# nmdl-mizo/lcaonet

Hardware: NVIDIA B200
Metric: molecules/sec fwd+bwd (QM9-shape) (higher is better)
Workload: dtype f32

## Files before the change

### lcaonet_b200/csrc/gemm_tc.cu

```cuda
#include "common.cuh"

namespace {

constexpr int kEpiWarps = 4;
constexpr int kBlockM = 128;
constexpr int kChunkK = 32;
constexpr uint32_t kSpinLimit = 1u << 28;

__device__ __forceinline__ uint32_t smem_u32(const void* p) { return (uint32_t)__cvta_generic_to_shared(p); }

__device__ __forceinline__ void mbar_init(uint64_t* bar, uint32_t count) {
  asm volatile("mbarrier.init.shared::cta.b64 [%0], %1;" ::"r"(smem_u32(bar)), "r"(count));
}
__device__ __forceinline__ void mbar_arrive(uint64_t* bar) {
  asm volatile("mbarrier.arrive.shared::cta.b64 _, [%0];" ::"r"(smem_u32(bar)) : "memory");
}
__device__ __forceinline__ void mbar_wait(uint64_t* bar, uint32_t parity) {
  uint32_t done = 0, spins = 0;
  const uint32_t addr = smem_u32(bar);
  while (!done) {
    asm volatile(
        "{\n\t.reg .pred p;\n\t"
        "mbarrier.try_wait.parity.shared::cta.b64 p, [%1], %2;\n\t"
        "selp.u32 %0, 1, 0, p;\n\t}"
        : "=r"(done)
        : "r"(addr), "r"(parity)
        : "memory");
    if (!done && ++spins > kSpinLimit) __trap();
  }
}
__device__ __forceinline__ void fence_barrier_init() { asm volatile("fence.mbarrier_init.release.cluster;" ::: "memory"); }
__device__ __forceinline__ void fence_proxy_async() { asm volatile("fence.proxy.async.shared::cta;" ::: "memory"); }
__device__ __forceinline__ void tc_fence_before() { asm volatile("tcgen05.fence::before_thread_sync;" ::: "memory"); }
__device__ __forceinline__ void tc_fence_after() { asm volatile("tcgen05.fence::after_thread_sync;" ::: "memory"); }

__device__ __forceinline__ void tmem_alloc(uint32_t* dst_smem, uint32_t ncols) {
  asm volatile("tcgen05.alloc.cta_group::1.sync.aligned.shared::cta.b32 [%0], %1;" ::"r"(smem_u32(dst_smem)), "r"(ncols)
               : "memory");
  asm volatile("tcgen05.relinquish_alloc_permit.cta_group::1.sync.aligned;" ::: "memory");
}
__device__ __forceinline__ void tmem_dealloc(uint32_t taddr, uint32_t ncols) {
  asm volatile("tcgen05.dealloc.cta_group::1.sync.aligned.b32 %0, %1;" ::"r"(taddr), "r"(ncols) : "memory");
}
__device__ __forceinline__ bool elect_one() {
  uint32_t pred;
  asm volatile("{\n\t.reg .pred p;\n\telect.sync _|p, 0xffffffff;\n\tselp.u32 %0, 1, 0, p;\n\t}" : "=r"(pred));
  return pred != 0;
}
__device__ __forceinline__ void umma_tf32(uint32_t tmem_d, uint64_t desc_a, uint64_t desc_b, uint32_t idesc,
                                          uint32_t accumulate) {
  asm volatile(
      "{\n\t.reg .pred p;\n\t"
      "setp.ne.b32 p, %4, 0;\n\t"
      "tcgen05.mma.cta_group::1.kind::tf32 [%0], %1, %2, %3, p;\n\t}"
      ::"r"(tmem_d), "l"(desc_a), "l"(desc_b), "r"(idesc), "r"(accumulate)
      : "memory");
}
__device__ __forceinline__ void umma_commit(uint64_t* bar) {
  asm volatile("tcgen05.commit.cta_group::1.mbarrier::arrive::one.shared::cluster.b64 [%0];" ::"r"(smem_u32(bar))
               : "memory");
}
__device__ __forceinline__ void tmem_ld32(uint32_t taddr, float (&v)[32]) {
  uint32_t r[32];
  asm volatile(
      "tcgen05.ld.sync.aligned.32x32b.x32.b32 "
      "{%0,%1,%2,%3,%4,%5,%6,%7,%8,%9,%10,%11,%12,%13,%14,%15,%16,%17,%18,%19,%20,%21,%22,%23,%24,%25,%26,%27,%28,%29,%30,%31}, [%32];"
      : "=r"(r[0]), "=r"(r[1]), "=r"(r[2]), "=r"(r[3]), "=r"(r[4]), "=r"(r[5]), "=r"(r[6]), "=r"(r[7]), "=r"(r[8]),
        "=r"(r[9]), "=r"(r[10]), "=r"(r[11]), "=r"(r[12]), "=r"(r[13]), "=r"(r[14]), "=r"(r[15]), "=r"(r[16]),
        "=r"(r[17]), "=r"(r[18]), "=r"(r[19]), "=r"(r[20]), "=r"(r[21]), "=r"(r[22]), "=r"(r[23]), "=r"(r[24]),
        "=r"(r[25]), "=r"(r[26]), "=r"(r[27]), "=r"(r[28]), "=r"(r[29]), "=r"(r[30]), "=r"(r[31])
      : "r"(taddr)
      : "memory");
  asm volatile("tcgen05.wait::ld.sync.aligned;" ::: "memory");
#pragma unroll
  for (int i = 0; i < 32; ++i) v[i] = __uint_as_float(r[i]);
}

__device__ __forceinline__ uint64_t make_desc_sw128(uint32_t smem_addr) {
  uint64_t d = 0;
  d |= (uint64_t)((smem_addr & 0x3FFFFu) >> 4);
  d |= (uint64_t)1 << 16;
  d |= (uint64_t)(1024 >> 4) << 32;
  d |= (uint64_t)1 << 46;
  d |= (uint64_t)2 << 61;
  return d;
}
__device__ __forceinline__ uint32_t sw128_off(int row, int chunk) { return row * 128 + ((chunk ^ (row & 7)) << 4); }
__host__ __device__ constexpr uint32_t make_idesc(int M, int N) {
  return (1u << 4) | (2u << 7) | (2u << 10) | ((uint32_t)(N >> 3) << 17) | ((uint32_t)(M >> 4) << 24);
}

__device__ __forceinline__ float tf32_hi(float x) { return __uint_as_float(__float_as_uint(x) & 0xFFFFE000u); }
__device__ __forceinline__ void split4(const float4 x, float4& hi, float4& lo) {
  hi = make_float4(tf32_hi(x.x), tf32_hi(x.y), tf32_hi(x.z), tf32_hi(x.w));
  lo = make_float4(tf32_hi(x.x - hi.x), tf32_hi(x.y - hi.y), tf32_hi(x.z - hi.z), tf32_hi(x.w - hi.w));
}
__device__ __forceinline__ float sigmoid_fast(float x) { return __fdividef(1.0f, 1.0f + __expf(-x)); }
__device__ __forceinline__ float silu_fast(float x) { return x * sigmoid_fast(x); }
__device__ __forceinline__ float silu_grad_fast(float x) {
  const float sg = sigmoid_fast(x);
  return sg * fmaf(x, 1.0f - sg, 1.0f);
}
__device__ __forceinline__ float4 silu_grad4(float4 g, float4 h) {
  return make_float4(g.x * silu_grad_fast(h.x), g.y * silu_grad_fast(h.y), g.z * silu_grad_fast(h.z), g.w * silu_grad_fast(h.w));
}

__device__ __forceinline__ void store8(float* p, const float* v, bool wide) {
  if (wide) {
    asm volatile("st.global.v8.f32 [%0], {%1,%2,%3,%4,%5,%6,%7,%8};" ::"l"(p), "f"(v[0]), "f"(v[1]), "f"(v[2]), "f"(v[3]),
                 "f"(v[4]), "f"(v[5]), "f"(v[6]), "f"(v[7])
                 : "memory");
  } else {
    st4(p, make_float4(v[0], v[1], v[2], v[3]));
    st4(p + 4, make_float4(v[4], v[5], v[6], v[7]));
  }
}

struct RowsArgs {
  const float* A; int64_t lda;
  const float* W; int64_t ldw;
  const float* bias;
  const float* G; int64_t ldg;
  float* Y; int64_t ldy;
  float* pre; int64_t ldp;
  int64_t M; int Kc; int Nb;
  int b_trans, act, accumulate, x3, stages, lo_stages;
  int wide_store;
};

constexpr int kLoadWarps = 4;
constexpr int kRowsThreads = (4 + 4 + 1 + kLoadWarps) * 32;
constexpr int kEpiPitch = 144;
constexpr int kEpiWarpBytes = 32 * kEpiPitch;
constexpr uint32_t kStageBytes = kBlockM * 128;

__device__ __forceinline__ void cp_async16(uint32_t dst, const void* src, uint32_t src_bytes) {
  asm volatile("cp.async.cg.shared.global [%0], [%1], 16, %2;" ::"r"(dst), "l"(src), "r"(src_bytes) : "memory");
}
__device__ __forceinline__ void cp_async_arrive(uint64_t* bar) {
  asm volatile("cp.async.mbarrier.arrive.noinc.shared::cta.b64 [%0];" ::"r"(smem_u32(bar)) : "memory");
}

template <bool EPI8>
__global__ void __launch_bounds__(EPI8 ? kRowsThreads + 128 : kRowsThreads, 1) k_tc_rows(const RowsArgs g) {
  extern __shared__ __align__(1024) uint8_t smem_raw[];
  pdl_trigger();
  const int warp = threadIdx.x >> 5, lane = threadIdx.x & 31;
  const uint32_t blockB = g.Nb * 128;
  const uint32_t halfB = (g.Kc / kChunkK) * blockB;
  const int R = g.stages, L = g.lo_stages;
  uint8_t* sB = smem_raw;
  uint8_t* sHi = sB + 2 * halfB;
  uint8_t* sLo = sHi + (size_t)R * kStageBytes;
  uint64_t* bars = reinterpret_cast<uint64_t*>(sLo + (size_t)(g.x3 ? L : 0) * kStageBytes);
  uint64_t* raw_full = bars;
  uint64_t* full = raw_full + R;
  uint64_t* hi_empty = full + R;
  uint64_t* lo_empty = hi_empty + R;
  uint64_t* tfull = lo_empty + L;
  uint64_t* tempty = tfull + 2;
  uint32_t* tmem_slot = reinterpret_cast<uint32_t*>(tempty + 2);

  const int64_t nblocks = (g.M + kBlockM - 1) / kBlockM;
  const int nchunk = g.Kc / kChunkK;
  const uint32_t acc_cols = g.x3 ? 2 * g.Nb : g.Nb;
  const uint32_t need_cols = 2 * acc_cols;
  const uint32_t tmem_cols = need_cols <= 32 ? 32 : need_cols <= 64 ? 64 : need_cols <= 128 ? 128 : need_cols <= 256 ? 256 : 512;

  if (threadIdx.x == 0) {
    for (int s = 0; s < R; ++s) {
      mbar_init(&raw_full[s], kLoadWarps * 32);
      mbar_init(&full[s], 4 * 32);
      mbar_init(&hi_empty[s], 1);
    }
    for (int s = 0; s < L; ++s) mbar_init(&lo_empty[s], 1);
    for (int a = 0; a < 2; ++a) {
      mbar_init(&tfull[a], 1);
      mbar_init(&tempty[a], (EPI8 ? 2 : 1) * kEpiWarps * 32);
    }
    fence_barrier_init();
  }
  if (warp == 8) tmem_alloc(tmem_slot, tmem_cols);
  tc_fence_before();
  __syncthreads();
  tc_fence_after();
  const uint32_t tmem_base = *tmem_slot;

  constexpr int kStageThreads = (4 + 4 + 1) * 32;
  constexpr int kWB = 8;
  if (warp < 9) {
    const int kq = g.Kc / 4, total = g.Nb * kq;
    for (int base = 0; base < total; base += kWB * kStageThreads) {
      float4 w[kWB];
      int n[kWB], kg[kWB];
#pragma unroll
      for (int u = 0; u < kWB; ++u) {
        const int idx = base + u * kStageThreads + (int)threadIdx.x;
        w[u] = make_float4(0.f, 0.f, 0.f, 0.f);
        n[u] = -1;
        if (idx < total) {
          if (!g.b_trans) {
            n[u] = idx / kq; kg[u] = idx - n[u] * kq;
            w[u] = ldg4(g.W + (int64_t)n[u] * g.ldw + kg[u] * 4);
          } else {
            kg[u] = idx / g.Nb; n[u] = idx - kg[u] * g.Nb;
            w[u] = make_float4(__ldg(g.W + (int64_t)(kg[u] * 4 + 0) * g.ldw + n[u]), __ldg(g.W + (int64_t)(kg[u] * 4 + 1) * g.ldw + n[u]),
                               __ldg(g.W + (int64_t)(kg[u] * 4 + 2) * g.ldw + n[u]), __ldg(g.W + (int64_t)(kg[u] * 4 + 3) * g.ldw + n[u]));
          }
        }
      }
#pragma unroll
      for (int u = 0; u < kWB; ++u) {
        if (n[u] >= 0) {
          float4 hi, lo;
          split4(w[u], hi, lo);
          const uint32_t off = (kg[u] >> 3) * blockB + sw128_off(n[u], kg[u] & 7);
          *reinterpret_cast<float4*>(sB + off) = hi;
          *reinterpret_cast<float4*>(sB + halfB + off) = lo;
        }
      }
    }
    fence_proxy_async();
    asm volatile("bar.sync 1, %0;" ::"n"(kStageThreads) : "memory");
  }

  pdl_wait();
  if (warp >= 9 && warp < 13) {
    const int lw = warp - 9, row_in = lane >> 3, c = lane & 7;
    const uint32_t hi_base = smem_u32(sHi);
    uint32_t it = 0;
    for (int64_t mb = blockIdx.x; mb < nblocks; mb += gridDim.x) {
      const int64_t mrow = mb * kBlockM + 32 * lw + row_in;
      for (int kc = 0; kc < nchunk; ++kc, ++it) {
        const int s = it % R;
        mbar_wait(&hi_empty[s], ((it / R) & 1) ^ 1);
        const uint32_t dst = hi_base + s * kStageBytes;
        const float* src = g.A + mrow * g.lda + kc * kChunkK + c * 4;
#pragma unroll
        for (int j = 0; j < 8; ++j) {
          const bool ok = mrow + 4 * j < g.M;
          cp_async16(dst + sw128_off(32 * lw + 4 * j + row_in, c), ok ? src + (int64_t)4 * j * g.lda : g.A, ok ? 16u : 0u);
        }
        cp_async_arrive(&raw_full[s]);
      }
    }
  } else if (warp >= 4 && warp < 8) {
    const int t = threadIdx.x - 128;
    uint32_t it = 0;
    for (int64_t mb = blockIdx.x; mb < nblocks; mb += gridDim.x) {
      for (int kc = 0; kc < nchunk; ++kc, ++it) {
        const int s = it % R, l = it % L;
        mbar_wait(&raw_full[s], (it / R) & 1);
        if (g.x3) {
          mbar_wait(&lo_empty[l], ((it / L) & 1) ^ 1);
          uint8_t* ph = sHi + (size_t)s * kStageBytes + t * 16;
          uint8_t* pl = sLo + (size_t)l * kStageBytes + t * 16;
#pragma unroll
          for (int i = 0; i < 8; ++i) {
            float4 hi, lo;
            split4(*reinterpret_cast<const float4*>(ph + i * 2048), hi, lo);
            *reinterpret_cast<float4*>(ph + i * 2048) = hi;
            *reinterpret_cast<float4*>(pl + i * 2048) = lo;
          }
        }
        fence_proxy_async();
        mbar_arrive(&full[s]);
      }
    }
  } else if (warp == 8) {
    {
      const uint32_t idesc = make_idesc(kBlockM, g.Nb);
      const uint32_t hiBase = smem_u32(sHi), loBase = smem_u32(sLo), bBase = smem_u32(sB);
      uint32_t it = 0, tile = 0;
      for (int64_t mb = blockIdx.x; mb < nblocks; mb += gridDim.x, ++tile) {
        const int acc = tile & 1;
        mbar_wait(&tempty[acc], ((tile >> 1) & 1) ^ 1);
        tc_fence_after();
        const uint32_t d = tmem_base + acc * acc_cols, dc = d + g.Nb;
        for (int kc = 0; kc < nchunk; ++kc, ++it) {
          const int s = it % R, l = it % L;
          mbar_wait(&full[s], (it / R) & 1);
          tc_fence_after();
          const uint32_t a_hi = hiBase + s * kStageBytes, a_lo = loBase + l * kStageBytes;
          const uint32_t b_hi = bBase + kc * blockB, b_lo = b_hi + halfB;
          const uint64_t dAh0 = make_desc_sw128(a_hi), dBh0 = make_desc_sw128(b_hi), dAl0 = make_desc_sw128(a_lo), dBl0 = make_desc_sw128(b_lo);
#pragma unroll
          for (int kk = 0; kk < kChunkK / 8; ++kk) {
            const uint64_t dAh = dAh0 + 2 * kk, dBh = dBh0 + 2 * kk, dAl = dAl0 + 2 * kk, dBl = dBl0 + 2 * kk;
            if (elect_one()) {
              umma_tf32(d, dAh, dBh, idesc, (kc | kk) != 0);
              if (g.x3) {
                umma_tf32(dc, dAl, dBh, idesc, (kc | kk) != 0);
                umma_tf32(dc, dAh, dBl, idesc, 1);
              }
            }
          }
          if (elect_one()) {
            umma_commit(&hi_empty[s]);
            if (g.x3) umma_commit(&lo_empty[l]);
          }
        }
        if (elect_one()) umma_commit(&tfull[acc]);
      }
    }
    __syncwarp();
  } else {
    const bool wide = g.wide_store != 0;
    const int quad = warp & 3;
    const int c_begin = (EPI8 && warp >= 13) ? 64 : 0, c_end = EPI8 ? min(g.Nb, c_begin + 64) : g.Nb;
    uint32_t tile = 0;
    for (int64_t mb = blockIdx.x; mb < nblocks; mb += gridDim.x, ++tile) {
      const int acc = tile & 1;
      const int64_t m = mb * kBlockM + quad * 32 + lane;
      float4 gq[8];
      if (g.G && m < g.M) {
#pragma unroll
        for (int q = 0; q < 8; ++q)
          gq[q] = (c_begin + 4 * q < g.Nb) ? ldg4(g.G + m * g.ldg + c_begin + 4 * q) : make_float4(0.f, 0.f, 0.f, 0.f);
      }
      mbar_wait(&tfull[acc], (tile >> 1) & 1);
      tc_fence_after();
      for (int c0 = c_begin; c0 < c_end; c0 += 32) {
        float4 gn[8];
        if (g.G && m < g.M && c0 + 32 < c_end) {
#pragma unroll
          for (int q = 0; q < 8; ++q)
            gn[q] = (c0 + 32 + 4 * q < g.Nb) ? ldg4(g.G + m * g.ldg + c0 + 32 + 4 * q) : make_float4(0.f, 0.f, 0.f, 0.f);
        }
        float v[32];
        tmem_ld32(tmem_base + ((uint32_t)(quad * 32) << 16) + acc * acc_cols + c0, v);
        if (g.x3) {
          float w[32];
          tmem_ld32(tmem_base + ((uint32_t)(quad * 32) << 16) + acc * acc_cols + g.Nb + c0, w);
#pragma unroll
          for (int j = 0; j < 32; ++j) v[j] += w[j];
        }
        if (m < g.M) {
          const int nc = min(32, g.Nb - c0);
#pragma unroll
          for (int j = 0; j < 32; j += 8) {
            if (j < nc) {
              float* o = v + j;
              if (g.bias) {
                const float4 b0 = ldg4(g.bias + c0 + j), b1 = ldg4(g.bias + c0 + j + 4);
                o[0] += b0.x; o[1] += b0.y; o[2] += b0.z; o[3] += b0.w; o[4] += b1.x; o[5] += b1.y; o[6] += b1.z; o[7] += b1.w;
              }
              if (g.accumulate) {
                const float4 p0 = *reinterpret_cast<const float4*>(g.Y + m * g.ldy + c0 + j);
                const float4 p1 = *reinterpret_cast<const float4*>(g.Y + m * g.ldy + c0 + j + 4);
                o[0] += p0.x; o[1] += p0.y; o[2] += p0.z; o[3] += p0.w; o[4] += p1.x; o[5] += p1.y; o[6] += p1.z; o[7] += p1.w;
              }
              if (g.pre) store8(g.pre + m * g.ldp + c0 + j, o, wide);
              if (g.act == LCAO_ACT_SILU) {
#pragma unroll
                for (int q = 0; q < 8; ++q) o[q] = silu_fast(o[q]);
              }
              if (g.G) {
                const float4 h0 = gq[j / 4], h1 = gq[j / 4 + 1];
                o[0] *= silu_grad_fast(h0.x); o[1] *= silu_grad_fast(h0.y); o[2] *= silu_grad_fast(h0.z); o[3] *= silu_grad_fast(h0.w);
                o[4] *= silu_grad_fast(h1.x); o[5] *= silu_grad_fast(h1.y); o[6] *= silu_grad_fast(h1.z); o[7] *= silu_grad_fast(h1.w);
              }
              store8(g.Y + m * g.ldy + c0 + j, o, wide);
            }
          }
        }
        if (g.G) {
#pragma unroll
          for (int q = 0; q < 8; ++q) gq[q] = gn[q];
        }
      }
      tc_fence_before();
      mbar_arrive(&tempty[acc]);
    }
  }
  tc_fence_before();
  __syncthreads();
  if (warp == 8) {
    tc_fence_after();
    tmem_dealloc(tmem_base, tmem_cols);
  }
}

constexpr int kTaThreads = 15 * 32;
constexpr int kTaStages = 4;
constexpr uint32_t kTaCol0 = 256;

__device__ __forceinline__ void umma_tf32_ts(uint32_t tmem_d, uint32_t tmem_a, uint64_t desc_b, uint32_t idesc, uint32_t accumulate) {
  asm volatile(
      "{\n\t.reg .pred p;\n\t"
      "setp.ne.b32 p, %4, 0;\n\t"
      "tcgen05.mma.cta_group::1.kind::tf32 [%0], [%1], %2, %3, p;\n\t}"
      ::"r"(tmem_d), "r"(tmem_a), "l"(desc_b), "r"(idesc), "r"(accumulate)
      : "memory");
}
__device__ __forceinline__ void tmem_st32(uint32_t taddr, const uint32_t (&r)[32]) {
  asm volatile(
      "tcgen05.st.sync.aligned.32x32b.x32.b32 [%0], "
      "{%1,%2,%3,%4,%5,%6,%7,%8,%9,%10,%11,%12,%13,%14,%15,%16,%17,%18,%19,%20,%21,%22,%23,%24,%25,%26,%27,%28,%29,%30,%31,%32};"
      ::"r"(taddr), "r"(r[0]), "r"(r[1]), "r"(r[2]), "r"(r[3]), "r"(r[4]), "r"(r[5]), "r"(r[6]), "r"(r[7]), "r"(r[8]), "r"(r[9]),
        "r"(r[10]), "r"(r[11]), "r"(r[12]), "r"(r[13]), "r"(r[14]), "r"(r[15]), "r"(r[16]), "r"(r[17]), "r"(r[18]), "r"(r[19]),
        "r"(r[20]), "r"(r[21]), "r"(r[22]), "r"(r[23]), "r"(r[24]), "r"(r[25]), "r"(r[26]), "r"(r[27]), "r"(r[28]), "r"(r[29]),
        "r"(r[30]), "r"(r[31])
      : "memory");
}
__device__ __forceinline__ void tmem_ld32_nw(uint32_t taddr, float (&v)[32]) {
  asm volatile(
      "tcgen05.ld.sync.aligned.32x32b.x32.b32 "
      "{%0,%1,%2,%3,%4,%5,%6,%7,%8,%9,%10,%11,%12,%13,%14,%15,%16,%17,%18,%19,%20,%21,%22,%23,%24,%25,%26,%27,%28,%29,%30,%31}, [%32];"
      : "=f"(v[0]), "=f"(v[1]), "=f"(v[2]), "=f"(v[3]), "=f"(v[4]), "=f"(v[5]), "=f"(v[6]), "=f"(v[7]), "=f"(v[8]),
        "=f"(v[9]), "=f"(v[10]), "=f"(v[11]), "=f"(v[12]), "=f"(v[13]), "=f"(v[14]), "=f"(v[15]), "=f"(v[16]),
        "=f"(v[17]), "=f"(v[18]), "=f"(v[19]), "=f"(v[20]), "=f"(v[21]), "=f"(v[22]), "=f"(v[23]), "=f"(v[24]),
        "=f"(v[25]), "=f"(v[26]), "=f"(v[27]), "=f"(v[28]), "=f"(v[29]), "=f"(v[30]), "=f"(v[31])
      : "r"(taddr)
      : "memory");
}
__device__ __forceinline__ void tmem_wait_ld() { asm volatile("tcgen05.wait::ld.sync.aligned;" ::: "memory"); }
__device__ __forceinline__ void tmem_wait_st() { asm volatile("tcgen05.wait::st.sync.aligned;" ::: "memory"); }

__global__ void __launch_bounds__(kTaThreads, 1) k_tc_rows_ta(const RowsArgs g) {
  constexpr int kLd = 2;
  extern __shared__ __align__(1024) uint8_t smem_raw[];
  pdl_trigger();
  const int warp = threadIdx.x >> 5, lane = threadIdx.x & 31;
  const uint32_t blockB = g.Nb * 128;
  const uint32_t halfB = (g.Kc / kChunkK) * blockB;
  const int R = g.stages;
  uint8_t* sB = smem_raw;
  uint8_t* sRaw = sB + 2 * halfB;
  uint64_t* bars = reinterpret_cast<uint64_t*>(sRaw + (size_t)R * kStageBytes);
  uint64_t* raw_full = bars;
  uint64_t* raw_empty = raw_full + R;
  uint64_t* a_full = raw_empty + R;
  uint64_t* a_empty = a_full + kTaStages;
  uint64_t* tfull = a_empty + kTaStages;
  uint64_t* tempty = tfull + 2;
  uint32_t* tmem_slot = reinterpret_cast<uint32_t*>(tempty + 2);
  const int64_t nblocks = (g.M + kBlockM - 1) / kBlockM;
  const int nchunk = g.Kc / kChunkK;
  constexpr uint32_t tmem_cols = 512;

  if (threadIdx.x == 0) {
    for (int s = 0; s < R; ++s) {
      mbar_init(&raw_full[s], kLd * 32);
      mbar_init(&raw_empty[s], 4 * 32);
    }
    for (int s = 0; s < kTaStages; ++s) {
      mbar_init(&a_full[s], 4 * 32);
      mbar_init(&a_empty[s], 1);
    }
    for (int a = 0; a < 2; ++a) {
      mbar_init(&tfull[a], 1);
      mbar_init(&tempty[a], 2 * kEpiWarps * 32);
    }
    fence_barrier_init();
  }
  if (warp == 8) tmem_alloc(tmem_slot, tmem_cols);
  tc_fence_before();
  __syncthreads();
  tc_fence_after();
  const uint32_t tmem_base = *tmem_slot;

  constexpr int kStageThreads = (4 + 4 + 1) * 32;
  constexpr int kWB = 8;
  if (warp < 9) {
    const int kq = g.Kc / 4, total = g.Nb * kq;
    for (int base = 0; base < total; base += kWB * kStageThreads) {
      float4 w[kWB];
      int n[kWB], kg[kWB];
#pragma unroll
      for (int u = 0; u < kWB; ++u) {
        const int idx = base + u * kStageThreads + (int)threadIdx.x;
        w[u] = make_float4(0.f, 0.f, 0.f, 0.f);
        n[u] = -1;
        if (idx < total) {
          if (!g.b_trans) {
            n[u] = idx / kq; kg[u] = idx - n[u] * kq;
            w[u] = ldg4(g.W + (int64_t)n[u] * g.ldw + kg[u] * 4);
          } else {
            kg[u] = idx / g.Nb; n[u] = idx - kg[u] * g.Nb;
            w[u] = make_float4(__ldg(g.W + (int64_t)(kg[u] * 4 + 0) * g.ldw + n[u]), __ldg(g.W + (int64_t)(kg[u] * 4 + 1) * g.ldw + n[u]),
                               __ldg(g.W + (int64_t)(kg[u] * 4 + 2) * g.ldw + n[u]), __ldg(g.W + (int64_t)(kg[u] * 4 + 3) * g.ldw + n[u]));
          }
        }
      }
#pragma unroll
      for (int u = 0; u < kWB; ++u) {
        if (n[u] >= 0) {
          float4 hi, lo;
          split4(w[u], hi, lo);
          const uint32_t off = (kg[u] >> 3) * blockB + sw128_off(n[u], kg[u] & 7);
          *reinterpret_cast<float4*>(sB + off) = hi;
          *reinterpret_cast<float4*>(sB + halfB + off) = lo;
        }
      }
    }
    fence_proxy_async();
    asm volatile("bar.sync 1, %0;" ::"n"(kStageThreads) : "memory");
  }
  pdl_wait();

  if (warp >= 9 && warp < 9 + kLd) {
    constexpr int kRowsPerLd = kBlockM / kLd;
    const int lw = warp - 9, row_in = lane >> 3, c = lane & 7;
    const uint32_t raw_base = smem_u32(sRaw);
    uint32_t it = 0;
    for (int64_t mb = blockIdx.x; mb < nblocks; mb += gridDim.x) {
      const int64_t mrow = mb * kBlockM + kRowsPerLd * lw + row_in;
      for (int kc = 0; kc < nchunk; ++kc, ++it) {
        const int s = it % R;
        mbar_wait(&raw_empty[s], ((it / R) & 1) ^ 1);
        const uint32_t dst = raw_base + s * kStageBytes;
        const float* src = g.A + mrow * g.lda + kc * kChunkK + c * 4;
#pragma unroll
        for (int j = 0; j < kRowsPerLd / 4; ++j) {
          const bool ok = mrow + 4 * j < g.M;
          cp_async16(dst + sw128_off(kRowsPerLd * lw + 4 * j + row_in, c), ok ? src + (int64_t)4 * j * g.lda : g.A, ok ? 16u : 0u);
        }
        cp_async_arrive(&raw_full[s]);
      }
    }
  } else if (warp >= 4 && warp < 8) {
    const int row = (warp & 3) * 32 + lane;
    const uint32_t lane_base = (uint32_t)((warp & 3) * 32) << 16;
    uint32_t it = 0;
    for (int64_t mb = blockIdx.x; mb < nblocks; mb += gridDim.x) {
      for (int kc = 0; kc < nchunk; ++kc, ++it) {
        const int s = it % R, ts = it % kTaStages;
        mbar_wait(&raw_full[s], (it / R) & 1);
        mbar_wait(&a_empty[ts], ((it / kTaStages) & 1) ^ 1);
        tc_fence_after();
        const uint8_t* pr = sRaw + (size_t)s * kStageBytes;
        uint32_t hi[32], lo[32];
#pragma unroll
        for (int c = 0; c < 8; ++c) {
          const float4 v = *reinterpret_cast<const float4*>(pr + sw128_off(row, c));
          float4 h, l;
          split4(v, h, l);
          hi[4 * c] = __float_as_uint(h.x); hi[4 * c + 1] = __float_as_uint(h.y); hi[4 * c + 2] = __float_as_uint(h.z); hi[4 * c + 3] = __float_as_uint(h.w);
          lo[4 * c] = __float_as_uint(l.x); lo[4 * c + 1] = __float_as_uint(l.y); lo[4 * c + 2] = __float_as_uint(l.z); lo[4 * c + 3] = __float_as_uint(l.w);
        }
        const uint32_t ta = tmem_base + lane_base + kTaCol0 + ts * 64;
        tmem_st32(ta, hi);
        tmem_st32(ta + 32, lo);
        mbar_arrive(&raw_empty[s]);
        tmem_wait_st();
        tc_fence_before();
        mbar_arrive(&a_full[ts]);
      }
    }
  } else if (warp == 8) {
    {
      const uint32_t idesc = make_idesc(kBlockM, g.Nb);
      const uint32_t bBase = smem_u32(sB);
      uint32_t it = 0, tile = 0;
      for (int64_t mb = blockIdx.x; mb < nblocks; mb += gridDim.x, ++tile) {
        const int acc = tile & 1;
        mbar_wait(&tempty[acc], ((tile >> 1) & 1) ^ 1);
        tc_fence_after();
        const uint32_t d = tmem_base + acc * g.Nb;
        for (int kc = 0; kc < nchunk; ++kc, ++it) {
          const int ts = it % kTaStages;
          mbar_wait(&a_full[ts], (it / kTaStages) & 1);
          tc_fence_after();
          const uint32_t a_hi = tmem_base + kTaCol0 + ts * 64, a_lo = a_hi + 32;
          const uint32_t b_hi = bBase + kc * blockB, b_lo = b_hi + halfB;
          const uint64_t dBh0 = make_desc_sw128(b_hi), dBl0 = make_desc_sw128(b_lo);
#pragma unroll
          for (int kk = 0; kk < kChunkK / 8; ++kk) {
            const uint64_t dBh = dBh0 + 2 * kk, dBl = dBl0 + 2 * kk;
            if (elect_one()) {
              umma_tf32_ts(d, a_hi + kk * 8, dBh, idesc, (kc | kk) != 0);
              umma_tf32_ts(d, a_lo + kk * 8, dBh, idesc, 1);
              umma_tf32_ts(d, a_hi + kk * 8, dBl, idesc, 1);
            }
          }
          if (elect_one()) umma_commit(&a_empty[ts]);
        }
        if (elect_one()) umma_commit(&tfull[acc]);
      }
    }
    __syncwarp();
  } else if (warp < 4 || warp >= 9 + kLd) {
    const bool wide = g.wide_store != 0;
    const int quad = warp & 3;
    const int c_begin = warp >= 9 + kLd ? 64 : 0, c_end = min(g.Nb, c_begin + 64);
    uint32_t tile = 0;
    for (int64_t mb = blockIdx.x; mb < nblocks; mb += gridDim.x, ++tile) {
      const int acc = tile & 1;
      const int64_t m = mb * kBlockM + quad * 32 + lane;
      mbar_wait(&tfull[acc], (tile >> 1) & 1);
      tc_fence_after();
      float v[2][32];
      const uint32_t t0 = tmem_base + ((uint32_t)(quad * 32) << 16) + acc * g.Nb;
      if (c_begin < c_end) tmem_ld32_nw(t0 + c_begin, v[0]);
      if (c_begin + 32 < c_end) tmem_ld32_nw(t0 + c_begin + 32, v[1]);
      tmem_wait_ld();
      tc_fence_before();
      mbar_arrive(&tempty[acc]);
      if (m < g.M) {
#pragma unroll
        for (int h = 0; h < 2; ++h) {
          const int c0 = c_begin + 32 * h;
          if (c0 < c_end) {
            const int nc = min(32, c_end - c0);
#pragma unroll
            for (int j = 0; j < 32; j += 8) {
              if (j < nc) {
                float* o = v[h] + j;
                if (g.bias) {
                  const float4 b0 = ldg4(g.bias + c0 + j), b1 = ldg4(g.bias + c0 + j + 4);
                  o[0] += b0.x; o[1] += b0.y; o[2] += b0.z; o[3] += b0.w; o[4] += b1.x; o[5] += b1.y; o[6] += b1.z; o[7] += b1.w;
                }
                if (g.accumulate) {
                  const float4 p0 = *reinterpret_cast<const float4*>(g.Y + m * g.ldy + c0 + j);
                  const float4 p1 = *reinterpret_cast<const float4*>(g.Y + m * g.ldy + c0 + j + 4);
                  o[0] += p0.x; o[1] += p0.y; o[2] += p0.z; o[3] += p0.w; o[4] += p1.x; o[5] += p1.y; o[6] += p1.z; o[7] += p1.w;
                }
                if (g.pre) store8(g.pre + m * g.ldp + c0 + j, o, wide);
                if (g.act == LCAO_ACT_SILU) {
#pragma unroll
                  for (int q = 0; q < 8; ++q) o[q] = silu_fast(o[q]);
                }
                if (g.G) {
                  const float4 h0 = ldg4(g.G + m * g.ldg + c0 + j), h1 = ldg4(g.G + m * g.ldg + c0 + j + 4);
                  o[0] *= silu_grad_fast(h0.x); o[1] *= silu_grad_fast(h0.y); o[2] *= silu_grad_fast(h0.z); o[3] *= silu_grad_fast(h0.w);
                  o[4] *= silu_grad_fast(h1.x); o[5] *= silu_grad_fast(h1.y); o[6] *= silu_grad_fast(h1.z); o[7] *= silu_grad_fast(h1.w);
                }
                store8(g.Y + m * g.ldy + c0 + j, o, wide);
              }
            }
          }
        }
      }
    }
  }
  tc_fence_before();
  __syncthreads();
  if (warp == 8) {
    tc_fence_after();
    tmem_dealloc(tmem_base, tmem_cols);
  }
}

struct WgradArgs {
  const float* dY; int64_t ldy;
  const float* X; int64_t ldx;
  float* dW; int64_t ldw;
  float* db;
  float* part;
  int64_t M; int Kx; int x3, raw_stages, op_stages;
};

__global__ void __launch_bounds__(kRowsThreads, 1) k_tc_wgrad(const WgradArgs g) {
  extern __shared__ __align__(1024) uint8_t smem_raw[];
  const int warp = threadIdx.x >> 5, lane = threadIdx.x & 31;
  const uint32_t rawA = kChunkK * 512, rawB = kChunkK * g.Kx * 4;
  const uint32_t opA = 128 * 128, opB = g.Kx * 128;
  const uint32_t op_stage = (g.x3 ? 2 : 1) * (opA + opB);
  const int Rr = g.raw_stages, S = g.op_stages;
  uint8_t* sOp = smem_raw;
  uint8_t* sRaw = sOp + (size_t)S * op_stage;
  uint64_t* bars = reinterpret_cast<uint64_t*>(sRaw + (size_t)Rr * (rawA + rawB));
  uint64_t* raw_full = bars;
  uint64_t* raw_empty = raw_full + Rr;
  uint64_t* op_full = raw_empty + Rr;
  uint64_t* op_empty = op_full + S;
  uint64_t* tfull = op_empty + S;
  uint64_t* tempty = tfull + 2;
  uint32_t* tmem_slot = reinterpret_cast<uint32_t*>(tempty + 2);
  constexpr int kFlush = 8;
  const uint32_t acc_cols = g.x3 ? 2 * g.Kx : g.Kx;
  const uint32_t need_cols = 2 * acc_cols;
  const uint32_t tmem_cols = need_cols <= 32 ? 32 : need_cols <= 64 ? 64 : need_cols <= 128 ? 128 : need_cols <= 256 ? 256 : 512;

  const int64_t nchunks = (g.M + kChunkK - 1) / kChunkK;
  const int64_t per = (nchunks + gridDim.x - 1) / gridDim.x;
  const int64_t c_beg = min(nchunks, (int64_t)blockIdx.x * per), c_end = min(nchunks, c_beg + per);

  if (threadIdx.x == 0) {
    for (int s = 0; s < Rr; ++s) {
      mbar_init(&raw_full[s], kLoadWarps * 32);
      mbar_init(&raw_empty[s], 4 * 32);
    }
    for (int s = 0; s < S; ++s) {
      mbar_init(&op_full[s], 4 * 32);
      mbar_init(&op_empty[s], 1);
    }
    for (int a = 0; a < 2; ++a) {
      mbar_init(&tfull[a], 1);
      mbar_init(&tempty[a], kEpiWarps * 32);
    }
    fence_barrier_init();
  }
  if (warp == 8) tmem_alloc(tmem_slot, tmem_cols);
  tc_fence_before();
  __syncthreads();
  tc_fence_after();
  const uint32_t tmem_base = *tmem_slot;
  pdl_trigger();
  pdl_wait();
  if (c_beg >= c_end) {
    for (int i = threadIdx.x; i < g.Kx * 128; i += kRowsThreads) g.part[(size_t)blockIdx.x * g.Kx * 128 + i] = 0.f;
    if (g.db && threadIdx.x < 128) g.part[(size_t)gridDim.x * g.Kx * 128 + (size_t)blockIdx.x * 128 + threadIdx.x] = 0.f;
    __syncthreads();
    if (warp == 8) tmem_dealloc(tmem_base, tmem_cols);
    return;
  }

  if (warp >= 9) {
    const int lw = warp - 9, r_in = lane >> 3, pl = lane & 7;
    const uint32_t raw_base = smem_u32(sRaw);
    const int pgB = g.Kx / 32;
    uint32_t it = 0;
    for (int64_t c = c_beg; c < c_end; ++c, ++it) {
      const int s = it % Rr;
      mbar_wait(&raw_empty[s], ((it / Rr) & 1) ^ 1);
      const uint32_t dA = raw_base + s * (rawA + rawB), dB = dA + rawA;
      const int64_t m0 = c * kChunkK;
#pragma unroll
      for (int j = 0; j < 8; ++j) {
        const int r = 8 * lw + (j & 1) * 4 + r_in, pg = j >> 1;
        const bool ok = m0 + r < g.M;
        cp_async16(dA + r * 512 + (((pg * 8 + pl) ^ (r >> 2)) << 4), ok ? g.dY + (m0 + r) * g.ldy + (pg * 8 + pl) * 4 : g.dY,
                   ok ? 16u : 0u);
      }
      for (int j = 0; j < 2 * pgB; ++j) {
        const int r = 8 * lw + (j & 1) * 4 + r_in, pg = j >> 1;
        const bool ok = m0 + r < g.M;
        cp_async16(dB + r * (g.Kx * 4) + (((pg * 8 + pl) ^ (r >> 2)) << 4), ok ? g.X + (m0 + r) * g.ldx + (pg * 8 + pl) * 4 : g.X,
                   ok ? 16u : 0u);
      }
      cp_async_arrive(&raw_full[s]);
    }
  } else if (warp >= 4 && warp < 8) {
    const int t = threadIdx.x - 128;
    const int kg = t & 7, g0 = t >> 3;
    const int ngB = g.Kx / 4;
    float4 colsum[2] = {make_float4(0.f, 0.f, 0.f, 0.f), make_float4(0.f, 0.f, 0.f, 0.f)};
    uint32_t it = 0;
    for (int64_t c = c_beg; c < c_end; ++c, ++it) {
      const int r = it % Rr, s = it % S;
      mbar_wait(&raw_full[r], (it / Rr) & 1);
      mbar_wait(&op_empty[s], ((it / S) & 1) ^ 1);
      const uint8_t* rA = sRaw + (size_t)r * (rawA + rawB);
      const uint8_t* rB = rA + rawA;
      uint8_t* oA = sOp + (size_t)s * op_stage;
      uint8_t* oB = oA + (g.x3 ? 2 : 1) * opA;
#pragma unroll
      for (int i = 0; i < 2; ++i) {
        const int ng = g0 + 16 * i;
        float4 v[4];
#pragma unroll
        for (int q = 0; q < 4; ++q) v[q] = *reinterpret_cast<const float4*>(rA + (4 * kg + q) * 512 + ((ng ^ kg) << 4));
#pragma unroll
        for (int q = 0; q < 4; ++q)
          colsum[i] = make_float4(colsum[i].x + v[q].x, colsum[i].y + v[q].y, colsum[i].z + v[q].z, colsum[i].w + v[q].w);
        const float4 col[4] = {make_float4(v[0].x, v[1].x, v[2].x, v[3].x), make_float4(v[0].y, v[1].y, v[2].y, v[3].y),
                               make_float4(v[0].z, v[1].z, v[2].z, v[3].z), make_float4(v[0].w, v[1].w, v[2].w, v[3].w)};
#pragma unroll
        for (int j = 0; j < 4; ++j) {
          float4 hi, lo;
          split4(col[j], hi, lo);
          const uint32_t off = sw128_off(4 * ng + j, kg);
          *reinterpret_cast<float4*>(oA + off) = hi;
          if (g.x3) *reinterpret_cast<float4*>(oA + opA + off) = lo;
        }
      }
      for (int ng = g0; ng < ngB; ng += 16) {
        float4 v[4];
#pragma unroll
        for (int q = 0; q < 4; ++q)
          v[q] = *reinterpret_cast<const float4*>(rB + (4 * kg + q) * (g.Kx * 4) + ((ng ^ kg) << 4));
        const float4 col[4] = {make_float4(v[0].x, v[1].x, v[2].x, v[3].x), make_float4(v[0].y, v[1].y, v[2].y, v[3].y),
                               make_float4(v[0].z, v[1].z, v[2].z, v[3].z), make_float4(v[0].w, v[1].w, v[2].w, v[3].w)};
#pragma unroll
        for (int j = 0; j < 4; ++j) {
          float4 hi, lo;
          split4(col[j], hi, lo);
          const uint32_t off = sw128_off(4 * ng + j, kg);
          *reinterpret_cast<float4*>(oB + off) = hi;
          if (g.x3) *reinterpret_cast<float4*>(oB + opB + off) = lo;
        }
      }
      fence_proxy_async();
      mbar_arrive(&op_full[s]);
      mbar_arrive(&raw_empty[r]);
    }
    if (g.db) {
#pragma unroll
      for (int i = 0; i < 2; ++i) {
        float4 c = colsum[i];
#pragma unroll
        for (int o = 1; o < 8; o <<= 1) {
          c.x += __shfl_xor_sync(0xffffffffu, c.x, o); c.y += __shfl_xor_sync(0xffffffffu, c.y, o);
          c.z += __shfl_xor_sync(0xffffffffu, c.z, o); c.w += __shfl_xor_sync(0xffffffffu, c.w, o);
        }
        if (kg == 0)
          *reinterpret_cast<float4*>(g.part + (size_t)gridDim.x * g.Kx * 128 + (size_t)blockIdx.x * 128 + (g0 + 16 * i) * 4) = c;
      }
    }
  } else if (warp == 8) {
    {
      const uint32_t idesc = make_idesc(kBlockM, g.Kx);
      const uint32_t base = smem_u32(sOp);
      uint32_t it = 0, fl = 0;
      for (int64_t c = c_beg; c < c_end; ++fl) {
        const int acc = fl & 1;
        mbar_wait(&tempty[acc], ((fl >> 1) & 1) ^ 1);
        tc_fence_after();
        const uint32_t d = tmem_base + acc * acc_cols, dc = d + g.Kx;
        const int64_t c_stop = min(c_end, c + kFlush);
        for (int first = 1; c < c_stop; ++c, ++it) {
          const int s = it % S;
          mbar_wait(&op_full[s], (it / S) & 1);
          tc_fence_after();
          const uint32_t a_hi = base + s * op_stage, a_lo = a_hi + opA, b_hi = a_hi + (g.x3 ? 2 : 1) * opA, b_lo = b_hi + opB;
          const uint64_t dAh0 = make_desc_sw128(a_hi), dBh0 = make_desc_sw128(b_hi), dAl0 = make_desc_sw128(a_lo), dBl0 = make_desc_sw128(b_lo);
#pragma unroll
          for (int kk = 0; kk < kChunkK / 8; ++kk) {
            const uint64_t dAh = dAh0 + 2 * kk, dBh = dBh0 + 2 * kk, dAl = dAl0 + 2 * kk, dBl = dBl0 + 2 * kk;
            if (elect_one()) {
              umma_tf32(d, dAh, dBh, idesc, !first);
              if (g.x3) {
                umma_tf32(dc, dAl, dBh, idesc, !first);
                umma_tf32(dc, dAh, dBl, idesc, 1);
              }
            }
            first = 0;
          }
          if (elect_one()) umma_commit(&op_empty[s]);
        }
        if (elect_one()) umma_commit(&tfull[acc]);
      }
    }
    __syncwarp();
  } else {
    constexpr int kMaxCols = 128;
    float sum[kMaxCols];
#pragma unroll
    for (int j = 0; j < kMaxCols; ++j) sum[j] = 0.f;
    const int64_t n_flush = (c_end - c_beg + kFlush - 1) / kFlush;
    for (int64_t fl = 0; fl < n_flush; ++fl) {
      const int acc = fl & 1;
      mbar_wait(&tfull[acc], (fl >> 1) & 1);
      tc_fence_after();
      const uint32_t t0 = tmem_base + ((uint32_t)(warp * 32) << 16) + acc * acc_cols;
#pragma unroll
      for (int c0 = 0; c0 < kMaxCols; c0 += 32) {
        if (c0 < g.Kx) {
          float v[32];
          tmem_ld32(t0 + c0, v);
#pragma unroll
          for (int j = 0; j < 32; ++j) sum[c0 + j] += v[j];
          if (g.x3) {
            tmem_ld32(t0 + g.Kx + c0, v);
#pragma unroll
            for (int j = 0; j < 32; ++j) sum[c0 + j] += v[j];
          }
        }
      }
      tc_fence_before();
      mbar_arrive(&tempty[acc]);
    }
    const int n = warp * 32 + lane;
    float* pp = g.part + (size_t)blockIdx.x * g.Kx * 128 + n;
#pragma unroll
    for (int j = 0; j < kMaxCols; ++j)
      if (j < g.Kx) pp[(size_t)j * 128] = sum[j];
  }
  tc_fence_before();
  __syncthreads();
  if (warp == 8) {
    tc_fence_after();
    tmem_dealloc(tmem_base, tmem_cols);
  }
}

__global__ void __launch_bounds__(1024) k_wgrad_reduce(const float* __restrict__ part, int ncta, int Kx, float* __restrict__ dW,
                                                       int64_t ldw, float* __restrict__ db) {
  __shared__ float s_p[8][128];
  pdl_trigger();
  pdl_wait();
  const int j = blockIdx.x, n = threadIdx.x & 127, ty = threadIdx.x >> 7;
  const bool bias_row = j >= Kx;
  const float* src = bias_row ? part + (size_t)ncta * Kx * 128 + n : part + (size_t)j * 128 + n;
  const size_t stride = bias_row ? 128 : (size_t)Kx * 128;
  float acc = 0.f;
  for (int c = ty; c < ncta; c += 8) acc += src[(size_t)c * stride];
  s_p[ty][n] = acc;
  __syncthreads();
  if (ty == 0) {
    const float t = ((s_p[0][n] + s_p[1][n]) + (s_p[2][n] + s_p[3][n])) + ((s_p[4][n] + s_p[5][n]) + (s_p[6][n] + s_p[7][n]));
    if (bias_row) db[n] += t;
    else dW[(int64_t)n * ldw + j] += t;
  }
}

struct WgradDesc { const float* part; float* dW; float* db; int64_t ldw; int ncta, Kx; };
constexpr int kMaxWgradBatch = 32;
struct WgradBatch { WgradDesc d[kMaxWgradBatch]; };
__global__ void __launch_bounds__(1024) k_wgrad_reduce_batch(const WgradBatch b) {
  __shared__ float s_p[8][128];
  pdl_trigger();
  pdl_wait();
  const WgradDesc& g = b.d[blockIdx.y];
  const int j = blockIdx.x, n = threadIdx.x & 127, ty = threadIdx.x >> 7;
  if (j > g.Kx || (j == g.Kx && !g.db)) return;
  const bool bias_row = j >= g.Kx;
  const float* src = bias_row ? g.part + (size_t)g.ncta * g.Kx * 128 + n : g.part + (size_t)j * 128 + n;
  const size_t stride = bias_row ? 128 : (size_t)g.Kx * 128;
  float acc = 0.f;
  for (int c = ty; c < g.ncta; c += 8) acc += src[(size_t)c * stride];
  s_p[ty][n] = acc;
  __syncthreads();
  if (ty == 0) {
    const float t = ((s_p[0][n] + s_p[1][n]) + (s_p[2][n] + s_p[3][n])) + ((s_p[4][n] + s_p[5][n]) + (s_p[6][n] + s_p[7][n]));
    if (bias_row) g.db[n] += t;
    else g.dW[(int64_t)n * g.ldw + j] += t;
  }
}

constexpr size_t kMaxSmem = 227 * 1024;

int num_sms() {
  static int n = 0;
  if (n == 0) {
    int dev = 0;
    cudaGetDevice(&dev);
    cudaDeviceGetAttribute(&n, cudaDevAttrMultiProcessorCount, dev);
    if (n <= 0) n = 148;
  }
  return n;
}

inline bool al16(const void* p) { return (reinterpret_cast<uintptr_t>(p) & 15u) == 0; }

}

static size_t rows_smem(int Kc, int Nb, int stages, int lo_stages) {
  const size_t halfB = (size_t)(Kc / kChunkK) * Nb * 128;
  return 2 * halfB + (size_t)(stages + lo_stages) * kStageBytes + 512 + 1024;
}

bool lcao_tc_rows_ok(int64_t M, int Kc, int Nb, int64_t lda, int64_t ldy, const void* A, const void* Y) {
  return M >= 512 && Kc % 32 == 0 && Kc >= 32 && Nb % 16 == 0 && Nb >= 16 && Nb <= 128 && lda % 4 == 0 && ldy % 4 == 0 &&
         al16(A) && al16(Y) && rows_smem(Kc, Nb, 2, 2) <= kMaxSmem;
}

int lcao_tc_rows(const float* A, int64_t lda, const float* W, int64_t ldw, int b_trans, const float* bias, const float* G,
                 int64_t ldg, float* Y, int64_t ldy, float* pre, int64_t ldp, int64_t M, int Kc, int Nb, int act,
                 int accumulate, int x3, cudaStream_t st) {
  RowsArgs g{};
  g.A = A; g.lda = lda; g.W = W; g.ldw = ldw; g.bias = bias; g.G = G; g.ldg = ldg; g.Y = Y; g.ldy = ldy;
  g.pre = pre; g.ldp = ldp; g.M = M; g.Kc = Kc; g.Nb = Nb; g.b_trans = b_trans; g.act = act; g.accumulate = accumulate;
  g.x3 = x3;
  g.wide_store = ((reinterpret_cast<uintptr_t>(Y) | (uintptr_t)(ldy * 4)) & 31u) == 0 &&
                 (!pre || ((reinterpret_cast<uintptr_t>(pre) | (uintptr_t)(ldp * 4)) & 31u) == 0);
  int lo_stages = x3 ? 3 : 0;
  int stages = 8;
  while (stages > 2 && rows_smem(Kc, Nb, stages, lo_stages) > kMaxSmem) --stages;
  if (x3 && stages < 3 && lo_stages > 2) {
    lo_stages = 2;
    stages = 8;
    while (stages > 2 && rows_smem(Kc, Nb, stages, lo_stages) > kMaxSmem) --stages;
  }
  g.stages = stages;
  g.lo_stages = x3 ? lo_stages : 1;
  const size_t smem = rows_smem(Kc, Nb, stages, lo_stages);
  static bool attr_set = false;
  if (!attr_set) {
    LCAO_CUDA(cudaFuncSetAttribute(k_tc_rows<false>, cudaFuncAttributeMaxDynamicSharedMemorySize, (int)kMaxSmem));
    LCAO_CUDA(cudaFuncSetAttribute(k_tc_rows<true>, cudaFuncAttributeMaxDynamicSharedMemorySize, (int)kMaxSmem));
    attr_set = true;
  }
  const int64_t nblocks = (M + kBlockM - 1) / kBlockM;
  const unsigned grid = (unsigned)(nblocks < num_sms() ? nblocks : num_sms());
  const bool epi8 = nblocks <= num_sms();
  if (x3 && nblocks >= 2 * num_sms() && Nb <= 128 && Kc % kChunkK == 0 &&
      2 * (size_t)(Kc / kChunkK) * Nb * 128 + 3 * kStageBytes + 512 + 1024 <= kMaxSmem) {
    static bool ta_attr = false;
    if (!ta_attr) {
      LCAO_CUDA(cudaFuncSetAttribute(k_tc_rows_ta, cudaFuncAttributeMaxDynamicSharedMemorySize, (int)kMaxSmem));
      ta_attr = true;
    }
    const size_t halfB = (size_t)(Kc / kChunkK) * Nb * 128;
    int R = 8;
    while (R > 2 && 2 * halfB + (size_t)R * kStageBytes + 512 + 1024 > kMaxSmem) --R;
    g.stages = R;
    const size_t smem_ta = 2 * halfB + (size_t)R * kStageBytes + 512 + 1024;
    LCAO_CUDA(launch_pdl(k_tc_rows_ta, grid, kTaThreads, smem_ta, st, g));
    LCAO_LAUNCH_CHECK();
    return LCAO_OK;
  }
  if (epi8) LCAO_CUDA(launch_pdl(k_tc_rows<true>, grid, kRowsThreads + 128, smem, st, g));
  else LCAO_CUDA(launch_pdl(k_tc_rows<false>, grid, kRowsThreads, smem, st, g));
  LCAO_LAUNCH_CHECK();
  return LCAO_OK;
}

static size_t wgrad_smem(int Kx, int x3, int raw_stages, int op_stages) {
  const size_t raw = (size_t)kChunkK * (512 + Kx * 4), op = (size_t)(x3 ? 2 : 1) * (128 * 128 + Kx * 128);
  return (size_t)raw_stages * raw + (size_t)op_stages * op + 512 + 1024;
}

bool lcao_tc_wgrad_ok(int64_t M, int Kx, int64_t ldy, int64_t ldx, const void* dY, const void* X) {
  return M >= 512 && Kx % 32 == 0 && Kx >= 32 && Kx <= 128 && ldy % 4 == 0 && ldx % 4 == 0 && al16(dY) && al16(X) &&
         wgrad_smem(Kx, 1, 2, 2) <= kMaxSmem;
}

static unsigned wgrad_grid(int64_t M) {
  const int64_t want = (M + 127) / 128;
  return (unsigned)(want < 1 ? 1 : want < num_sms() ? want : num_sms());
}
int64_t lcao_tc_wgrad_scratch(int64_t M, int Kx) { return (int64_t)wgrad_grid(M) * ((int64_t)Kx * 128 + 128); }

int lcao_tc_wgrad(const float* dY, int64_t ldy, const float* X, int64_t ldx, float* dW, int64_t ldw, float* db, int64_t M,
                  int Kx, int x3, float* part, cudaStream_t st, int64_t* defer_desc) {
  WgradArgs g{};
  g.dY = dY; g.ldy = ldy; g.X = X; g.ldx = ldx; g.dW = dW; g.ldw = ldw; g.db = db; g.part = part;
  g.M = M; g.Kx = Kx; g.x3 = x3;
  g.op_stages = 2;
  int raw_stages = 6;
  while (raw_stages > 2 && wgrad_smem(Kx, x3, raw_stages, g.op_stages) > kMaxSmem) --raw_stages;
  g.raw_stages = raw_stages;
  static bool attr_set = false;
  if (!attr_set) {
    LCAO_CUDA(cudaFuncSetAttribute(k_tc_wgrad, cudaFuncAttributeMaxDynamicSharedMemorySize, (int)kMaxSmem));
    attr_set = true;
  }
  const unsigned grid = wgrad_grid(M);
  LCAO_CUDA(launch_pdl(k_tc_wgrad, grid, kRowsThreads, wgrad_smem(Kx, x3, raw_stages, g.op_stages), st, g));
  LCAO_LAUNCH_CHECK();
  if (defer_desc) {
    defer_desc[0] = (int64_t)(uintptr_t)part; defer_desc[1] = (int64_t)(uintptr_t)dW; defer_desc[2] = (int64_t)(uintptr_t)db;
    defer_desc[3] = ldw; defer_desc[4] = (int64_t)grid; defer_desc[5] = Kx;
    return LCAO_OK;
  }
  LCAO_CUDA(launch_pdl(k_wgrad_reduce, Kx + (db ? 1 : 0), 1024, 0, st, (const float*)part, (int)grid, Kx, dW, ldw, db));
  LCAO_LAUNCH_CHECK();
  return LCAO_OK;
}

int lcao_tc_wgrad_reduce_batch(const int64_t* desc, int n, cudaStream_t st) {
  for (int i0 = 0; i0 < n; i0 += kMaxWgradBatch) {
    WgradBatch b{};
    const int m = n - i0 < kMaxWgradBatch ? n - i0 : kMaxWgradBatch;
    int kmax = 0;
    for (int i = 0; i < m; ++i) {
      const int64_t* d = desc + 6 * (int64_t)(i0 + i);
      b.d[i].part = reinterpret_cast<const float*>((uintptr_t)d[0]);
      b.d[i].dW = reinterpret_cast<float*>((uintptr_t)d[1]);
      b.d[i].db = reinterpret_cast<float*>((uintptr_t)d[2]);
      b.d[i].ldw = d[3]; b.d[i].ncta = (int)d[4]; b.d[i].Kx = (int)d[5];
      kmax = b.d[i].Kx > kmax ? b.d[i].Kx : kmax;
    }
    LCAO_CUDA(launch_pdl(k_wgrad_reduce_batch, dim3((unsigned)(kmax + 1), (unsigned)m), 1024, 0, st, b));
    LCAO_LAUNCH_CHECK();
  }
  return LCAO_OK;
}
```

Measured before the change: 113,500.

## Feed wgrad UMMA directly from raw tiles via MN-major swizzled descriptors

The weight-gradient tcgen05 kernel now loads dY and X straight into an MN-major SW128 layout that the MMA reads directly, using MN-major instruction and smem descriptors. This removes the transpose-and-copy of the hi operand into a separate staging buffer. The transform warps now only compute the TF32 lo residuals for the 3xTF32 path plus the bias column sums. Raw-stage release moves from transform-warp arrivals to an MMA commit. This cuts shared-memory traffic and transform work, but correctness depends on the new swizzle offsets and descriptor strides matching the hardware's MN-major layout exactly.

```diff
diff --git a/lcaonet_b200/csrc/gemm_tc.cu b/lcaonet_b200/csrc/gemm_tc.cu
--- a/lcaonet_b200/csrc/gemm_tc.cu
+++ b/lcaonet_b200/csrc/gemm_tc.cu
@@ -86,8 +86,22 @@
   return d;
 }
 __device__ __forceinline__ uint32_t sw128_off(int row, int chunk) { return row * 128 + ((chunk ^ (row & 7)) << 4); }
-__host__ __device__ constexpr uint32_t make_idesc(int M, int N) {
-  return (1u << 4) | (2u << 7) | (2u << 10) | ((uint32_t)(N >> 3) << 17) | ((uint32_t)(M >> 4) << 24);
+__device__ __forceinline__ uint64_t make_desc_mn_sw128(uint32_t smem_addr) {
+  uint64_t d = 0;
+  d |= (uint64_t)((smem_addr & 0x3FFFFu) >> 4);
+  d |= (uint64_t)(4096 >> 4) << 16;
+  d |= (uint64_t)(512 >> 4) << 32;
+  d |= (uint64_t)1 << 46;
+  d |= (uint64_t)1 << 61;
+  return d;
+}
+__device__ __forceinline__ uint32_t mn_off(int k, int pc) {
+  return (uint32_t)(pc >> 3) * 4096u + (uint32_t)(k >> 2) * 512u + (uint32_t)(k & 3) * 128u +
+         ((uint32_t)(((pc & 7) >> 1) ^ (k & 3)) << 5) + (uint32_t)(pc & 1) * 16u;
+}
+__host__ __device__ constexpr uint32_t make_idesc(int M, int N, int mn_major = 0) {
+  return (1u << 4) | (2u << 7) | (2u << 10) | ((uint32_t)mn_major << 15) | ((uint32_t)mn_major << 16) |
+         ((uint32_t)(N >> 3) << 17) | ((uint32_t)(M >> 4) << 24);
 }
 
 __device__ __forceinline__ float tf32_hi(float x) { return __uint_as_float(__float_as_uint(x) & 0xFFFFE000u); }
@@ -654,13 +668,12 @@
 __global__ void __launch_bounds__(kRowsThreads, 1) k_tc_wgrad(const WgradArgs g) {
   extern __shared__ __align__(1024) uint8_t smem_raw[];
   const int warp = threadIdx.x >> 5, lane = threadIdx.x & 31;
-  const uint32_t rawA = kChunkK * 512, rawB = kChunkK * g.Kx * 4;
   const uint32_t opA = 128 * 128, opB = g.Kx * 128;
-  const uint32_t op_stage = (g.x3 ? 2 : 1) * (opA + opB);
+  const uint32_t raw_stage = opA + opB, lo_stage = g.x3 ? opA + opB : 0;
   const int Rr = g.raw_stages, S = g.op_stages;
-  uint8_t* sOp = smem_raw;
-  uint8_t* sRaw = sOp + (size_t)S * op_stage;
-  uint64_t* bars = reinterpret_cast<uint64_t*>(sRaw + (size_t)Rr * (rawA + rawB));
+  uint8_t* sRaw = smem_raw;
+  uint8_t* sLo = sRaw + (size_t)Rr * raw_stage;
+  uint64_t* bars = reinterpret_cast<uint64_t*>(sLo + (size_t)S * lo_stage);
   uint64_t* raw_full = bars;
   uint64_t* raw_empty = raw_full + Rr;
   uint64_t* op_full = raw_empty + Rr;
@@ -680,7 +693,7 @@
   if (threadIdx.x == 0) {
     for (int s = 0; s < Rr; ++s) {
       mbar_init(&raw_full[s], kLoadWarps * 32);
-      mbar_init(&raw_empty[s], 4 * 32);
+      mbar_init(&raw_empty[s], 1);
     }
     for (int s = 0; s < S; ++s) {
       mbar_init(&op_full[s], 4 * 32);
@@ -715,94 +728,84 @@
     for (int64_t c = c_beg; c < c_end; ++c, ++it) {
       const int s = it % Rr;
       mbar_wait(&raw_empty[s], ((it / Rr) & 1) ^ 1);
-      const uint32_t dA = raw_base + s * (rawA + rawB), dB = dA + rawA;
+      const uint32_t dA = raw_base + s * raw_stage, dB = dA + opA;
       const int64_t m0 = c * kChunkK;
 #pragma unroll
       for (int j = 0; j < 8; ++j) {
         const int r = 8 * lw + (j & 1) * 4 + r_in, pg = j >> 1;
         const bool ok = m0 + r < g.M;
-        cp_async16(dA + r * 512 + (((pg * 8 + pl) ^ (r >> 2)) << 4), ok ? g.dY + (m0 + r) * g.ldy + (pg * 8 + pl) * 4 : g.dY,
-                   ok ? 16u : 0u);
+        cp_async16(dA + mn_off(r, pg * 8 + pl), ok ? g.dY + (m0 + r) * g.ldy + (pg * 8 + pl) * 4 : g.dY, ok ? 16u : 0u);
       }
       for (int j = 0; j < 2 * pgB; ++j) {
         const int r = 8 * lw + (j & 1) * 4 + r_in, pg = j >> 1;
         const bool ok = m0 + r < g.M;
-        cp_async16(dB + r * (g.Kx * 4) + (((pg * 8 + pl) ^ (r >> 2)) << 4), ok ? g.X + (m0 + r) * g.ldx + (pg * 8 + pl) * 4 : g.X,
+        cp_async16(dB + mn_off(r, pg * 8 + pl), ok ? g.X + (m0 + r) * g.ldx + (pg * 8 + pl) * 4 : g.X,
                    ok ? 16u : 0u);
       }
       cp_async_arrive(&raw_full[s]);
     }
   } else if (warp >= 4 && warp < 8) {
-    const int t = threadIdx.x - 128;
-    const int kg = t & 7, g0 = t >> 3;
-    const int ngB = g.Kx / 4;
+    const int w = warp - 4, kh = lane >> 3, pl = lane & 7;
+    const int pcA = 8 * w + pl, pgB = g.Kx / 32;
     float4 colsum[2] = {make_float4(0.f, 0.f, 0.f, 0.f), make_float4(0.f, 0.f, 0.f, 0.f)};
     uint32_t it = 0;
     for (int64_t c = c_beg; c < c_end; ++c, ++it) {
       const int r = it % Rr, s = it % S;
       mbar_wait(&raw_full[r], (it / Rr) & 1);
       mbar_wait(&op_empty[s], ((it / S) & 1) ^ 1);
-      const uint8_t* rA = sRaw + (size_t)r * (rawA + rawB);
-      const uint8_t* rB = rA + rawA;
-      uint8_t* oA = sOp + (size_t)s * op_stage;
-      uint8_t* oB = oA + (g.x3 ? 2 : 1) * opA;
-#pragma unroll
-      for (int i = 0; i < 2; ++i) {
-        const int ng = g0 + 16 * i;
-        float4 v[4];
-#pragma unroll
-        for (int q = 0; q < 4; ++q) v[q] = *reinterpret_cast<const float4*>(rA + (4 * kg + q) * 512 + ((ng ^ kg) << 4));
-#pragma unroll
-        for (int q = 0; q < 4; ++q)
-          colsum[i] = make_float4(colsum[i].x + v[q].x, colsum[i].y + v[q].y, colsum[i].z + v[q].z, colsum[i].w + v[q].w);
-        const float4 col[4] = {make_float4(v[0].x, v[1].x, v[2].x, v[3].x), make_float4(v[0].y, v[1].y, v[2].y, v[3].y),
-                               make_float4(v[0].z, v[1].z, v[2].z, v[3].z), make_float4(v[0].w, v[1].w, v[2].w, v[3].w)};
-#pragma unroll
-        for (int j = 0; j < 4; ++j) {
+      const uint8_t* rA = sRaw + (size_t)r * raw_stage;
+      const uint8_t* rB = rA + opA;
+      uint8_t* lA = sLo + (size_t)s * lo_stage;
+      uint8_t* lB = lA + opA;
+      float4 va[8], vb[8];
+#pragma unroll
+      for (int i = 0; i < 8; ++i) va[i] = *reinterpret_cast<const float4*>(rA + mn_off(4 * (kh + 4 * (i >> 2)) + (i & 3), pcA));
+      if (g.x3) {
+#pragma unroll
+        for (int j = 0; j < 8; ++j)
+          if (j < 2 * pgB) vb[j] = *reinterpret_cast<const float4*>(rB + mn_off(4 * w + kh + 16 * (j & 1), (j >> 1) * 8 + pl));
+      }
+#pragma unroll
+      for (int i = 0; i < 8; ++i) {
+        const float4 v = va[i];
+        colsum[i >> 2] = make_float4(colsum[i >> 2].x + v.x, colsum[i >> 2].y + v.y, colsum[i >> 2].z + v.z, colsum[i >> 2].w + v.w);
+        if (g.x3) {
           float4 hi, lo;
-          split4(col[j], hi, lo);
-          const uint32_t off = sw128_off(4 * ng + j, kg);
-          *reinterpret_cast<float4*>(oA + off) = hi;
-          if (g.x3) *reinterpret_cast<float4*>(oA + opA + off) = lo;
-        }
-      }
-      for (int ng = g0; ng < ngB; ng += 16) {
-        float4 v[4];
-#pragma unroll
-        for (int q = 0; q < 4; ++q)
-          v[q] = *reinterpret_cast<const float4*>(rB + (4 * kg + q) * (g.Kx * 4) + ((ng ^ kg) << 4));
-        const float4 col[4] = {make_float4(v[0].x, v[1].x, v[2].x, v[3].x), make_float4(v[0].y, v[1].y, v[2].y, v[3].y),
-                               make_float4(v[0].z, v[1].z, v[2].z, v[3].z), make_float4(v[0].w, v[1].w, v[2].w, v[3].w)};
-#pragma unroll
-        for (int j = 0; j < 4; ++j) {
-          float4 hi, lo;
-          split4(col[j], hi, lo);
-          const uint32_t off = sw128_off(4 * ng + j, kg);
-          *reinterpret_cast<float4*>(oB + off) = hi;
-          if (g.x3) *reinterpret_cast<float4*>(oB + opB + off) = lo;
+          split4(v, hi, lo);
+          *reinterpret_cast<float4*>(lA + mn_off(4 * (kh + 4 * (i >> 2)) + (i & 3), pcA)) = lo;
+        }
+      }
+      if (g.x3) {
+#pragma unroll
+        for (int j = 0; j < 8; ++j) {
+          if (j < 2 * pgB) {
+            float4 hi, lo;
+            split4(vb[j], hi, lo);
+            *reinterpret_cast<float4*>(lB + mn_off(4 * w + kh + 16 * (j & 1), (j >> 1) * 8 + pl)) = lo;
+          }
         }
       }
       fence_proxy_async();
       mbar_arrive(&op_full[s]);
-      mbar_arrive(&raw_empty[r]);
     }
     if (g.db) {
 #pragma unroll
       for (int i = 0; i < 2; ++i) {
-        float4 c = colsum[i];
-#pragma unroll
-        for (int o = 1; o < 8; o <<= 1) {
+#pragma unroll
+        for (int o = 8; o < 32; o <<= 1) {
+          float4& c = colsum[i];
           c.x += __shfl_xor_sync(0xffffffffu, c.x, o); c.y += __shfl_xor_sync(0xffffffffu, c.y, o);
           c.z += __shfl_xor_sync(0xffffffffu, c.z, o); c.w += __shfl_xor_sync(0xffffffffu, c.w, o);
         }
-        if (kg == 0)
-          *reinterpret_cast<float4*>(g.part + (size_t)gridDim.x * g.Kx * 128 + (size_t)blockIdx.x * 128 + (g0 + 16 * i) * 4) = c;
-      }
+      }
+      if (kh == 0)
+        *reinterpret_cast<float4*>(g.part + (size_t)gridDim.x * g.Kx * 128 + (size_t)blockIdx.x * 128 + pcA * 4) =
+            make_float4(colsum[0].x + colsum[1].x, colsum[0].y + colsum[1].y, colsum[0].z + colsum[1].z, colsum[0].w + colsum[1].w);
     }
   } else if (warp == 8) {
     {
-      const uint32_t idesc = make_idesc(kBlockM, g.Kx);
-      const uint32_t base = smem_u32(sOp);
+      const uint32_t idesc = make_idesc(kBlockM, g.Kx, 1);
+      const uint32_t rbase = smem_u32(sRaw), lbase = smem_u32(sLo);
       uint32_t it = 0, fl = 0;
       for (int64_t c = c_beg; c < c_end; ++fl) {
         const int acc = fl & 1;
@@ -811,14 +814,15 @@
         const uint32_t d = tmem_base + acc * acc_cols, dc = d + g.Kx;
         const int64_t c_stop = min(c_end, c + kFlush);
         for (int first = 1; c < c_stop; ++c, ++it) {
-          const int s = it % S;
+          const int r = it % Rr, s = it % S;
           mbar_wait(&op_full[s], (it / S) & 1);
           tc_fence_after();
-          const uint32_t a_hi = base + s * op_stage, a_lo = a_hi + opA, b_hi = a_hi + (g.x3 ? 2 : 1) * opA, b_lo = b_hi + opB;
-          const uint64_t dAh0 = make_desc_sw128(a_hi), dBh0 = make_desc_sw128(b_hi), dAl0 = make_desc_sw128(a_lo), dBl0 = make_desc_sw128(b_lo);
+          const uint32_t a_hi = rbase + r * raw_stage, b_hi = a_hi + opA, a_lo = lbase + s * lo_stage, b_lo = a_lo + opA;
+          const uint64_t dAh0 = make_desc_mn_sw128(a_hi), dBh0 = make_desc_mn_sw128(b_hi), dAl0 = make_desc_mn_sw128(a_lo),
+                         dBl0 = make_desc_mn_sw128(b_lo);
 #pragma unroll
           for (int kk = 0; kk < kChunkK / 8; ++kk) {
-            const uint64_t dAh = dAh0 + 2 * kk, dBh = dBh0 + 2 * kk, dAl = dAl0 + 2 * kk, dBl = dBl0 + 2 * kk;
+            const uint64_t dAh = dAh0 + 64 * kk, dBh = dBh0 + 64 * kk, dAl = dAl0 + 64 * kk, dBl = dBl0 + 64 * kk;
             if (elect_one()) {
               umma_tf32(d, dAh, dBh, idesc, !first);
               if (g.x3) {
@@ -828,7 +832,10 @@
             }
             first = 0;
           }
-          if (elect_one()) umma_commit(&op_empty[s]);
+          if (elect_one()) {
+            umma_commit(&raw_empty[r]);
+            umma_commit(&op_empty[s]);
+          }
         }
         if (elect_one()) umma_commit(&tfull[acc]);
       }
@@ -999,8 +1006,8 @@
 }
 
 static size_t wgrad_smem(int Kx, int x3, int raw_stages, int op_stages) {
-  const size_t raw = (size_t)kChunkK * (512 + Kx * 4), op = (size_t)(x3 ? 2 : 1) * (128 * 128 + Kx * 128);
-  return (size_t)raw_stages * raw + (size_t)op_stages * op + 512 + 1024;
+  const size_t tile = (size_t)128 * 128 + (size_t)Kx * 128;
+  return (size_t)raw_stages * tile + (size_t)op_stages * (x3 ? tile : 0) + 512 + 1024;
 }
 
 bool lcao_tc_wgrad_ok(int64_t M, int Kx, int64_t ldy, int64_t ldx, const void* dY, const void* X) {
```

Result: no change. 114,200 (median of 6 runs) (+0.6%).
